# scanner-research/scanner

Measured on AMD Instinct MI355X. Metric: frames/sec (whole node), 1080p histogram + ResNet-50 classify pipelines, higher is better.
Workload: dtype bf16; 1 GPU; model=1080p histogram + ResNet-50 classify, global_batch=512, seq_len=512, parallelism=frame-shard dp1

## Files before the change

### scanner_amd/kernels/gemm_mfma.hip

```cpp
#include <hip/hip_runtime.h>

#include <algorithm>
#include <cstdlib>
#include <map>
#include <mutex>

#include "../csrc/memory.h"
#include "dnn.h"

namespace sca {

namespace {

using bf16 = __bf16;
using bf16x8 = __attribute__((ext_vector_type(8))) __bf16;
using f32x4 = __attribute__((ext_vector_type(4))) float;

__device__ inline float bf16_to_f32(bf16 v) { return (float)v; }

__device__ inline bf16 f32_to_bf16(float v) { return (bf16)v; }

template <int FM, int FN, bool RELU, bool RESIDUAL>
__device__ inline void epilogue_store(f32x4 (&acc)[FM][FN], float* scratch,
                                      bf16* __restrict__ C,
                                      const bf16* __restrict__ residual,
                                      int M, int N, int m0, int n0, int wrow,
                                      int wcol, int lane,
                                      const float* __restrict__ scale,
                                      const float* __restrict__ bias) {
  constexpr int COLS = FN * 16;
  constexpr int STRIDE = COLS + 4;
#pragma unroll
  for (int i = 0; i < FM; ++i) {
    asm volatile("s_waitcnt lgkmcnt(0)");
#pragma unroll
    for (int j = 0; j < FN; ++j) {
      int cw = j * 16 + (lane & 15);
      int col = n0 + wcol * COLS + cw;
      float sc = scale ? scale[col] : 1.f;
      float bi = bias ? bias[col] : 0.f;
#pragma unroll
      for (int r = 0; r < 4; ++r) {
        scratch[((lane >> 4) * 4 + r) * STRIDE + cw] =
            acc[i][j][r] * sc + bi;
      }
    }
    asm volatile("s_waitcnt lgkmcnt(0)");
    constexpr int CHUNK = COLS / 4;
    static_assert(CHUNK >= 8 && CHUNK % 8 == 0, "wave tile too narrow");
    int r2 = lane >> 2;
    int q = lane & 3;
    int row = m0 + wrow * (FM * 16) + i * 16 + r2;
    if (row < M) {
      int colbase = n0 + wcol * COLS + q * CHUNK;
      const float* src = scratch + r2 * STRIDE + q * CHUNK;
      bf16 out[CHUNK];
#pragma unroll
      for (int k = 0; k < CHUNK; ++k) {
        float v = src[k];
        if constexpr (RESIDUAL) {
          v += bf16_to_f32(residual[(size_t)row * N + colbase + k]);
        }
        if constexpr (RELU) v = v > 0.f ? v : 0.f;
        out[k] = f32_to_bf16(v);
      }
#pragma unroll
      for (int c8 = 0; c8 < CHUNK; c8 += 8) {
        *reinterpret_cast<bf16x8*>(C + (size_t)row * N + colbase + c8) =
            *reinterpret_cast<const bf16x8*>(out + c8);
      }
    }
  }
}

template <int BM, int BN, int WM, int WN, bool RELU, bool RESIDUAL,
          bool IMPLICIT>
__global__ void __launch_bounds__(256, 2)
    gemm_bf16_kernel(const bf16* __restrict__ A, const bf16* __restrict__ B,
                     bf16* __restrict__ C, int M, int N, int K,
                     const float* __restrict__ scale,
                     const float* __restrict__ bias,
                     const bf16* __restrict__ residual, ConvDesc d,
                     const bf16* __restrict__ zero) {
  constexpr int BK = 64;
  constexpr int FM = BM / WM / 16;
  constexpr int FN = BN / WN / 16;
  __shared__ bf16 lds[2 * (BM + BN) * BK];

  int tid = threadIdx.x;
  int lane = tid & 63;
  int wave = tid >> 6;
  int wrow = wave / WN;
  int wcol = wave % WN;

  int nwg = gridDim.x;
  int wgid = blockIdx.x;
  if (nwg % 8 == 0) {
    int q = nwg / 8;
    wgid = (wgid % q) * 8 + wgid / q;
  }
  int ntiles_n = (N + BN - 1) / BN;
  int m0 = (wgid / ntiles_n) * BM;
  int n0 = (wgid % ntiles_n) * BN;

  f32x4 acc[FM][FN];
#pragma unroll
  for (int i = 0; i < FM; ++i)
#pragma unroll
    for (int j = 0; j < FN; ++j) acc[i][j] = f32x4{0.f, 0.f, 0.f, 0.f};

  constexpr int A_INSTRS = BM / 8 / 4;
  constexpr int B_INSTRS = BN / 8 / 4;
  const int lrow = lane >> 3;
  const int lk = (lane & 7) * 8;
  i64 imp_rowbase[IMPLICIT ? A_INSTRS : 1];
  int imp_hh0[IMPLICIT ? A_INSTRS : 1];
  int imp_ww0[IMPLICIT ? A_INSTRS : 1];
  int imp_cell = 0, imp_cj = 0, imp_dr = 0, imp_ds = 0;
  if constexpr (IMPLICIT) {
#pragma unroll
    for (int i = 0; i < A_INSTRS; ++i) {
      int row = (wave * A_INSTRS + i) * 8 + lrow;
      int grow = m0 + row;
      if (grow >= M) grow = M - 1;
      int q = grow % d.ow;
      int t = grow / d.ow;
      int p = t % d.oh;
      int nn = t / d.oh;
      imp_rowbase[i] = (i64)nn * d.h * d.w * d.c;
      imp_hh0[i] = p * d.stride - d.pad;
      imp_ww0[i] = q * d.stride - d.pad;
    }
    imp_cell = lk / d.c;
    imp_cj = lk - imp_cell * d.c;
    imp_dr = imp_cell / d.s;
    imp_ds = imp_cell - imp_dr * d.s;
  }
  auto imp_advance = [&](int dk) {
    imp_cj += dk;
    while (imp_cj >= d.c) {
      imp_cj -= d.c;
      ++imp_cell;
      ++imp_ds;
      if (imp_ds == d.s) {
        imp_ds = 0;
        ++imp_dr;
      }
    }
  };
  auto stage = [&](int buf, int k0) {
    bf16* lds_a = lds + buf * (BM + BN) * BK;
    bf16* lds_b = lds_a + BM * BK;
#pragma unroll
    for (int i = 0; i < A_INSTRS; ++i) {
      int row = (wave * A_INSTRS + i) * 8 + lrow;
      int grow = m0 + row;
      if (grow >= M) grow = M - 1;
      const bf16* src;
      if constexpr (IMPLICIT) {
        if (imp_cell >= d.r * d.s) {
          src = zero;
        } else {
          int hh = imp_hh0[i] + imp_dr;
          int ww = imp_ww0[i] + imp_ds;
          src = (hh >= 0 && hh < d.h && ww >= 0 && ww < d.w)
                    ? A + (imp_rowbase[i] + ((i64)hh * d.w + ww) * d.c +
                           imp_cj)
                    : zero;
        }
      } else {
        src = A + (size_t)grow * K + k0 + lk;
      }
      __builtin_amdgcn_global_load_lds(
          (const __attribute__((address_space(1))) uint32_t*)src,
          (__attribute__((address_space(3)))
               uint32_t*)(lds_a + (size_t)(wave * A_INSTRS + i) * 8 * BK),
          16, 0, 0);
    }
#pragma unroll
    for (int i = 0; i < B_INSTRS; ++i) {
      int row = (wave * B_INSTRS + i) * 8 + lrow;
      const bf16* src = B + (size_t)(n0 + row) * K + k0 + lk;
      __builtin_amdgcn_global_load_lds(
          (const __attribute__((address_space(1))) uint32_t*)src,
          (__attribute__((address_space(3)))
               uint32_t*)(lds_b + (size_t)(wave * B_INSTRS + i) * 8 * BK),
          16, 0, 0);
    }
  };

  int ksteps = K / BK;
  stage(0, 0);
  for (int ks = 0; ks < ksteps; ++ks) {
    int buf = ks & 1;
    __builtin_amdgcn_s_waitcnt( 0);
    __syncthreads();
    if (ks + 1 < ksteps) {
      if constexpr (IMPLICIT) imp_advance(BK);
      stage(buf ^ 1, (ks + 1) * BK);
    }

    const bf16* lds_a = lds + buf * (BM + BN) * BK;
    const bf16* lds_b = lds_a + BM * BK;
#pragma unroll
    for (int kk = 0; kk < 2; ++kk) {
      int kbase = kk * 32 + (lane >> 4) * 8;
      bf16x8 afrag[FM], bfrag[FN];
#pragma unroll
      for (int i = 0; i < FM; ++i) {
        int row = wrow * (BM / WM) + i * 16 + (lane & 15);
        afrag[i] = *reinterpret_cast<const bf16x8*>(
            lds_a + (size_t)row * BK + kbase);
      }
#pragma unroll
      for (int j = 0; j < FN; ++j) {
        int col = wcol * (BN / WN) + j * 16 + (lane & 15);
        bfrag[j] = *reinterpret_cast<const bf16x8*>(
            lds_b + (size_t)col * BK + kbase);
      }
#pragma unroll
      for (int i = 0; i < FM; ++i)
#pragma unroll
        for (int j = 0; j < FN; ++j)
          acc[i][j] = __builtin_amdgcn_mfma_f32_16x16x32_bf16(
              afrag[i], bfrag[j], acc[i][j], 0, 0, 0);
    }
  }

  __syncthreads();
  constexpr int EP_STRIDE = BN / WN + 4;
  float* scratch =
      reinterpret_cast<float*>(lds) + (size_t)wave * 16 * EP_STRIDE;
  epilogue_store<FM, FN, RELU, RESIDUAL>(acc, scratch, C, residual, M, N,
                                         m0, n0, wrow, wcol, lane, scale,
                                         bias);
}

template <int BM, int BN, int WM, int WN, bool RELU, bool RESIDUAL>
__global__ void __launch_bounds__(256, 2)
    gemm_bf16_smallk_kernel(const bf16* __restrict__ A,
                            const bf16* __restrict__ B, bf16* __restrict__ C,
                            int M, int N, const float* __restrict__ scale,
                            const float* __restrict__ bias,
                            const bf16* __restrict__ residual,
                            int tiles_per_wg) {
  constexpr int K = 64;
  constexpr int FM = BM / WM / 16;
  constexpr int FN = BN / WN / 16;
  __shared__ bf16 lds_b[BN * K];
  __shared__ bf16 lds_a[2 * BM * K];
  __shared__ float lds_ep[4 * 16 * (BN / WN + 4)];

  int tid = threadIdx.x;
  int lane = tid & 63;
  int wave = tid >> 6;
  int wrow = wave / WN;
  int wcol = wave % WN;

  int ntiles_n = (N + BN - 1) / BN;
  int ntiles_m = (M + BM - 1) / BM;
  int strip = blockIdx.x / ntiles_n;
  int n0 = (blockIdx.x % ntiles_n) * BN;
  int mt0 = strip * tiles_per_wg;
  int mt_end = min(mt0 + tiles_per_wg, ntiles_m);
  if (mt0 >= ntiles_m) return;

  const int lrow = lane >> 3;
  const int lk = (lane & 7) * 8;
  constexpr int B_INSTRS = BN / 8 / 4;
  constexpr int A_INSTRS = BM / 8 / 4;

#pragma unroll
  for (int i = 0; i < B_INSTRS; ++i) {
    int row = (wave * B_INSTRS + i) * 8 + lrow;
    const bf16* src = B + (size_t)(n0 + row) * K + lk;
    __builtin_amdgcn_global_load_lds(
        (const __attribute__((address_space(1))) uint32_t*)src,
        (__attribute__((address_space(3)))
             uint32_t*)(lds_b + (size_t)(wave * B_INSTRS + i) * 8 * K),
        16, 0, 0);
  }

  auto stage_a = [&](int buf, int mt) {
    int m0 = mt * BM;
    bf16* dst = lds_a + buf * BM * K;
#pragma unroll
    for (int i = 0; i < A_INSTRS; ++i) {
      int row = (wave * A_INSTRS + i) * 8 + lrow;
      int grow = m0 + row;
      if (grow >= M) grow = M - 1;
      const bf16* src = A + (size_t)grow * K + lk;
      __builtin_amdgcn_global_load_lds(
          (const __attribute__((address_space(1))) uint32_t*)src,
          (__attribute__((address_space(3)))
               uint32_t*)(dst + (size_t)(wave * A_INSTRS + i) * 8 * K),
          16, 0, 0);
    }
  };

  stage_a(0, mt0);
  for (int mt = mt0; mt < mt_end; ++mt) {
    int buf = (mt - mt0) & 1;
    __builtin_amdgcn_s_waitcnt(0);
    __syncthreads();
    if (mt + 1 < mt_end) stage_a(buf ^ 1, mt + 1);

    f32x4 acc[FM][FN];
#pragma unroll
    for (int i = 0; i < FM; ++i)
#pragma unroll
      for (int j = 0; j < FN; ++j) acc[i][j] = f32x4{0.f, 0.f, 0.f, 0.f};
// ... 11 lines not shown
      }
#pragma unroll
      for (int j = 0; j < FN; ++j) {
        int col = wcol * (BN / WN) + j * 16 + (lane & 15);
        bfrag[j] = *reinterpret_cast<const bf16x8*>(lds_b +
                                                    (size_t)col * K + kbase);
      }
#pragma unroll
      for (int i = 0; i < FM; ++i)
#pragma unroll
        for (int j = 0; j < FN; ++j)
          acc[i][j] = __builtin_amdgcn_mfma_f32_16x16x32_bf16(
              afrag[i], bfrag[j], acc[i][j], 0, 0, 0);
    }

    epilogue_store<FM, FN, RELU, RESIDUAL>(
        acc, lds_ep + (size_t)wave * 16 * (BN / WN + 4), C, residual, M, N,
        mt * BM, n0, wrow, wcol, lane, scale, bias);
  }
}

struct SplitkEp {
  unsigned int* counters = nullptr;
  int splits = 0;
  const float* scale = nullptr;
  const float* bias = nullptr;
  const bf16* residual = nullptr;
  bf16* C = nullptr;
  int relu = 0;
};

template <int BM, int BN, int WM, int WN, bool IMPLICIT, bool ATOMIC>
__global__ void __launch_bounds__(256, 2)
    gemm_bf16_splitk_kernel(const bf16* __restrict__ A,
                            const bf16* __restrict__ B, int M, int N, int K,
                            int ksteps_per_split,
                            float* __restrict__ partials, ConvDesc d,
                            const bf16* __restrict__ zero, SplitkEp ep) {
  constexpr int BK = 64;
  constexpr int FM = BM / WM / 16;
  constexpr int FN = BN / WN / 16;
  __shared__ bf16 lds[2 * (BM + BN) * BK];

  int tid = threadIdx.x;
  int lane = tid & 63;
  int wave = tid >> 6;
  int wrow = wave / WN;
// ... 4 lines not shown
  int tiles = ntiles_m * ntiles_n;
  int split = blockIdx.x / tiles;
  int tile = blockIdx.x % tiles;
  int m0 = (tile / ntiles_n) * BM;
  int n0 = (tile % ntiles_n) * BN;
  int ks_begin = split * ksteps_per_split;
  int ks_end = min(ks_begin + ksteps_per_split, K / BK);
  if (ks_begin >= ks_end) return;

  f32x4 acc[FM][FN];
#pragma unroll
  for (int i = 0; i < FM; ++i)
#pragma unroll
    for (int j = 0; j < FN; ++j) acc[i][j] = f32x4{0.f, 0.f, 0.f, 0.f};

  constexpr int A_INSTRS = BM / 8 / 4;
  constexpr int B_INSTRS = BN / 8 / 4;
  auto stage = [&](int buf, int k0) {
    const int lrow = lane >> 3;
    const int lk = (lane & 7) * 8;
    bf16* lds_a = lds + buf * (BM + BN) * BK;
    bf16* lds_b = lds_a + BM * BK;
#pragma unroll
    for (int i = 0; i < A_INSTRS; ++i) {
      int row = (wave * A_INSTRS + i) * 8 + lrow;
      int grow = m0 + row;
      if (grow >= M) grow = M - 1;
      const bf16* src;
      if constexpr (IMPLICIT) {
        int k = k0 + lk;
        int cell = k / d.c;
        int cj = k - cell * d.c;
        if (cell >= d.r * d.s) {
          src = zero;
        } else {
          int dr = cell / d.s, ds = cell - dr * d.s;
          int q = grow % d.ow;
          int t = grow / d.ow;
          int p = t % d.oh;
          int nn = t / d.oh;
          int hh = p * d.stride - d.pad + dr;
          int ww = q * d.stride - d.pad + ds;
          src = (hh >= 0 && hh < d.h && ww >= 0 && ww < d.w)
                    ? A + ((((i64)nn * d.h + hh) * d.w + ww) * d.c + cj)
                    : zero;
        }
      } else {
        src = A + (size_t)grow * K + k0 + lk;
      }
      __builtin_amdgcn_global_load_lds(
          (const __attribute__((address_space(1))) uint32_t*)src,
          (__attribute__((address_space(3)))
               uint32_t*)(lds_a + (size_t)(wave * A_INSTRS + i) * 8 * BK),
          16, 0, 0);
    }
#pragma unroll
    for (int i = 0; i < B_INSTRS; ++i) {
      int row = (wave * B_INSTRS + i) * 8 + lrow;
      const bf16* src = B + (size_t)(n0 + row) * K + k0 + lk;
      __builtin_amdgcn_global_load_lds(
          (const __attribute__((address_space(1))) uint32_t*)src,
          (__attribute__((address_space(3)))
               uint32_t*)(lds_b + (size_t)(wave * B_INSTRS + i) * 8 * BK),
          16, 0, 0);
    }
  };

  stage(0, ks_begin * BK);
  for (int ks = ks_begin; ks < ks_end; ++ks) {
    int buf = (ks - ks_begin) & 1;
    __builtin_amdgcn_s_waitcnt(0);
    __syncthreads();
    if (ks + 1 < ks_end) stage(buf ^ 1, (ks + 1) * BK);

    const bf16* lds_a = lds + buf * (BM + BN) * BK;
    const bf16* lds_b = lds_a + BM * BK;
#pragma unroll
    for (int kk = 0; kk < 2; ++kk) {
      int kbase = kk * 32 + (lane >> 4) * 8;
      bf16x8 afrag[FM], bfrag[FN];
#pragma unroll
      for (int i = 0; i < FM; ++i) {
        int row = wrow * (BM / WM) + i * 16 + (lane & 15);
        afrag[i] = *reinterpret_cast<const bf16x8*>(
            lds_a + (size_t)row * BK + kbase);
      }
#pragma unroll
      for (int j = 0; j < FN; ++j) {
        int col = wcol * (BN / WN) + j * 16 + (lane & 15);
        bfrag[j] = *reinterpret_cast<const bf16x8*>(
            lds_b + (size_t)col * BK + kbase);
      }
#pragma unroll
      for (int i = 0; i < FM; ++i)
#pragma unroll
        for (int j = 0; j < FN; ++j)
          acc[i][j] = __builtin_amdgcn_mfma_f32_16x16x32_bf16(
              afrag[i], bfrag[j], acc[i][j], 0, 0, 0);
    }
    __syncthreads();
  }

  if constexpr (ATOMIC) {
#pragma unroll
    for (int i = 0; i < FM; ++i) {
#pragma unroll
      for (int j = 0; j < FN; ++j) {
        int col = n0 + wcol * (BN / WN) + j * 16 + (lane & 15);
#pragma unroll
        for (int r = 0; r < 4; ++r) {
          int row = m0 + wrow * (BM / WM) + i * 16 + (lane >> 4) * 4 + r;
          if (row < M)
            atomicAdd(&partials[(size_t)row * N + col], acc[i][j][r]);
        }
      }
// ... 3 lines not shown
#pragma unroll
    for (int i = 0; i < FM; ++i) {
#pragma unroll
      for (int j = 0; j < FN; ++j) {
        int col = n0 + wcol * (BN / WN) + j * 16 + (lane & 15);
#pragma unroll
        for (int r = 0; r < 4; ++r) {
          int row = m0 + wrow * (BM / WM) + i * 16 + (lane >> 4) * 4 + r;
          if (row < M) out[(size_t)row * N + col] = acc[i][j][r];
        }
      }
    }
    if (ep.counters) {
      __threadfence();
      __syncthreads();
      __shared__ unsigned int s_old;
      if (tid == 0) s_old = atomicAdd(ep.counters + tile, 1u);
      __syncthreads();
      if (s_old != (unsigned int)ep.splits - 1) return;
      __threadfence();
      int rows = min(BM, M - m0);
      constexpr int Q = BN / 4;
      for (int idx = tid; idx < rows * Q; idx += 256) {
        int r = idx / Q, q = idx - r * Q;
        size_t base = (size_t)(m0 + r) * N + n0 + q * 4;
        float4 av = make_float4(0.f, 0.f, 0.f, 0.f);
        for (int sp = 0; sp < ep.splits; ++sp) {
          float4 p = *reinterpret_cast<const float4*>(
              partials + (size_t)sp * M * N + base);
          av.x += p.x;
          av.y += p.y;
          av.z += p.z;
          av.w += p.w;
        }
        float v4[4] = {av.x, av.y, av.z, av.w};
        bf16 o4[4];
#pragma unroll
        for (int k = 0; k < 4; ++k) {
          float v = v4[k];
          int col = n0 + q * 4 + k;
          if (ep.scale) v *= ep.scale[col];
          if (ep.bias) v += ep.bias[col];
          if (ep.residual) v += bf16_to_f32(ep.residual[base + k]);
          if (ep.relu) v = v > 0.f ? v : 0.f;
          o4[k] = f32_to_bf16(v);
        }
        *reinterpret_cast<uint64_t*>(ep.C + base) =
            *reinterpret_cast<const uint64_t*>(o4);
      }
      if (tid == 0) ep.counters[tile] = 0;
    }
  }
}

template <bool RELU, bool RESIDUAL>
__global__ void __launch_bounds__(256)
    splitk_finalize_kernel(const float* __restrict__ acc, i64 mn, int N,
                           const float* __restrict__ scale,
                           const float* __restrict__ bias,
                           const bf16* __restrict__ residual,
                           bf16* __restrict__ C) {
  i64 quads = mn / 4;
  i64 gs = (i64)gridDim.x * blockDim.x;
  for (i64 q = (i64)blockIdx.x * blockDim.x + threadIdx.x; q < quads;
       q += gs) {
    i64 i = q * 4;
    float4 a4 = reinterpret_cast<const float4*>(acc)[q];
    float v4[4] = {a4.x, a4.y, a4.z, a4.w};
    bf16 o4[4];
#pragma unroll
    for (int k = 0; k < 4; ++k) {
      float v = v4[k];
      int col = (int)((i + k) % N);
      if (scale) v *= scale[col];
      if (bias) v += bias[col];
      if constexpr (RESIDUAL) v += bf16_to_f32(residual[i + k]);
      if constexpr (RELU) v = v > 0.f ? v : 0.f;
      o4[k] = f32_to_bf16(v);
    }
    *reinterpret_cast<uint64_t*>(C + i) =
        *reinterpret_cast<const uint64_t*>(o4);
  }
}

template <bool RELU, bool RESIDUAL>
__global__ void __launch_bounds__(256)
    splitk_reduce_kernel(const float* __restrict__ partials, int splits,
                         i64 mn, int N, const float* __restrict__ scale,
                         const float* __restrict__ bias,
                         const bf16* __restrict__ residual,
                         bf16* __restrict__ C) {
  i64 quads = mn / 4;
  i64 gs = (i64)gridDim.x * blockDim.x;
  for (i64 q = (i64)blockIdx.x * blockDim.x + threadIdx.x; q < quads;
       q += gs) {
    i64 i = q * 4;
    float4 acc = make_float4(0.f, 0.f, 0.f, 0.f);
    for (int sp = 0; sp < splits; ++sp) {
      float4 p = reinterpret_cast<const float4*>(
          partials + (size_t)sp * mn)[q];
      acc.x += p.x;
      acc.y += p.y;
      acc.z += p.z;
      acc.w += p.w;
    }
    float v4[4] = {acc.x, acc.y, acc.z, acc.w};
    bf16 o4[4];
#pragma unroll
    for (int k = 0; k < 4; ++k) {
      float v = v4[k];
      int col = (int)((i + k) % N);
      if (scale) v *= scale[col];
      if (bias) v += bias[col];
      if constexpr (RESIDUAL) v += bf16_to_f32(residual[i + k]);
      if constexpr (RELU) v = v > 0.f ? v : 0.f;
      o4[k] = f32_to_bf16(v);
    }
    *reinterpret_cast<uint64_t*>(C + i) =
        *reinterpret_cast<const uint64_t*>(o4);
  }
}

const bf16* device_zero_chunk();

constexpr size_t kSplitkCtrBytes = 4096;

bool plan_splitk(int M, int N, int K, size_t scratch_bytes, GemmPlan& p) {
  constexpr int BM = 128, BN = 128;
  static const bool kOff = []() {
    const char* e = std::getenv("SCANNER_SPLITK_OFF");
    return e && e[0] == '1';
  }();
  if (kOff) return false;
  if (!scratch_bytes || N % BN != 0 || K < 1024) return false;
  int ntiles_m = (M + BM - 1) / BM;
  int tiles = ntiles_m * (N / BN);
  if (tiles >= 256) return false;
  static const int kMaxSplits = []() {
// ... 43 lines not shown
        (u8*)g.splitk_scratch + g.splitk_scratch_bytes - kSplitkCtrBytes);
    ep.splits = splits;
    ep.scale = g.scale;
    ep.bias = g.bias;
    ep.residual = (const bf16*)g.residual;
    ep.C = (bf16*)g.C;
    ep.relu = g.relu ? 1 : 0;
  }
  hipError_t e;
  if (kAtomic) {
    e = hipMemsetAsync(g.splitk_scratch, 0, (size_t)mn * 4, s);
    if (e != hipSuccess) {
      throw ScannerError(std::string("splitk memset failed: ") +
                         hipGetErrorString(e));
    }
    if (dd) {
      gemm_bf16_splitk_kernel<BM, BN, 2, 2, true, true>
          <<<grid_main, 256, 0, s>>>(
              (const bf16*)g.A, (const bf16*)g.B, g.M, g.N, g.K,
              ksteps_per_split, (float*)g.splitk_scratch, *dd,
              device_zero_chunk(), SplitkEp{});
    } else {
      gemm_bf16_splitk_kernel<BM, BN, 2, 2, false, true>
          <<<grid_main, 256, 0, s>>>(
              (const bf16*)g.A, (const bf16*)g.B, g.M, g.N, g.K,
              ksteps_per_split, (float*)g.splitk_scratch, ConvDesc{},
              nullptr, SplitkEp{});
    }
  } else if (dd) {
    gemm_bf16_splitk_kernel<BM, BN, 2, 2, true, false>
        <<<grid_main, 256, 0, s>>>(
            (const bf16*)g.A, (const bf16*)g.B, g.M, g.N, g.K,
            ksteps_per_split, (float*)g.splitk_scratch, *dd,
            device_zero_chunk(), ep);
  } else {
    gemm_bf16_splitk_kernel<BM, BN, 2, 2, false, false>
        <<<grid_main, 256, 0, s>>>(
            (const bf16*)g.A, (const bf16*)g.B, g.M, g.N, g.K,
            ksteps_per_split, (float*)g.splitk_scratch, ConvDesc{}, nullptr,
            ep);
  }
  e = hipGetLastError();
  if (e != hipSuccess) {
    throw ScannerError(std::string("splitk launch failed: ") +
                       hipGetErrorString(e));
  }
  if (fused) return;
  int grid = (int)std::min<i64>(4096, (mn + 255) / 256);
  auto disp = [&](auto relu, auto res) {
    if (kAtomic) {
      splitk_finalize_kernel<decltype(relu)::value, decltype(res)::value>
          <<<grid, 256, 0, s>>>((const float*)g.splitk_scratch, mn, g.N,
                                g.scale, g.bias, (const bf16*)g.residual,
                                (bf16*)g.C);
    } else {
      splitk_reduce_kernel<decltype(relu)::value, decltype(res)::value>
          <<<grid, 256, 0, s>>>((const float*)g.splitk_scratch, splits, mn,
                                g.N, g.scale, g.bias,
                                (const bf16*)g.residual, (bf16*)g.C);
    }
  };
  if (g.relu && g.residual)
    disp(std::true_type{}, std::true_type{});
  else if (g.relu)
    disp(std::true_type{}, std::false_type{});
  else if (g.residual)
    disp(std::false_type{}, std::true_type{});
  else
    disp(std::false_type{}, std::false_type{});
  e = hipGetLastError();
  if (e != hipSuccess) {
    throw ScannerError(std::string("splitk reduce launch failed: ") +
                       hipGetErrorString(e));
  }
// ... 33 lines not shown
    disp(std::false_type{}, std::true_type{});
  else
    disp(std::false_type{}, std::false_type{});
  hipError_t e = hipGetLastError();
  if (e != hipSuccess) {
    throw ScannerError(std::string("gemm smallk launch failed: ") +
                       hipGetErrorString(e));
  }
}

template <int BM, int BN, int WM, int WN>
void launch_variant(const GemmArgs& g, hipStream_t s, const GemmPlan& p) {
  const int grid = p.grid;
  auto disp = [&](auto relu, auto res) {
    gemm_bf16_kernel<BM, BN, WM, WN, decltype(relu)::value,
                     decltype(res)::value, false><<<grid, 256, 0, s>>>(
        (const bf16*)g.A, (const bf16*)g.B, (bf16*)g.C, g.M, g.N, g.K,
        g.scale, g.bias, (const bf16*)g.residual, ConvDesc{}, nullptr);
  };
  if (g.relu && g.residual)
    disp(std::true_type{}, std::true_type{});
  else if (g.relu)
    disp(std::true_type{}, std::false_type{});
  else if (g.residual)
    disp(std::false_type{}, std::true_type{});
  else
    disp(std::false_type{}, std::false_type{});
  hipError_t e = hipGetLastError();
  if (e != hipSuccess) {
    throw ScannerError(std::string("gemm launch failed: ") +
                       hipGetErrorString(e));
// ... 10 lines not shown
  if (it != per_dev.end()) return it->second;
  void* p = nullptr;
  hipError_t e = hipMalloc(&p, 256);
  if (e != hipSuccess || hipMemset(p, 0, 256) != hipSuccess) {
    throw ScannerError("failed to allocate implicit-conv zero chunk");
  }
  per_dev[dev] = (bf16*)p;
  return (bf16*)p;
}

template <int BM, int BN, int WM, int WN>
void launch_conv_variant(const GemmArgs& g, const ConvDesc& d,
                         hipStream_t s, const GemmPlan& p) {
  const int grid = p.grid;
  const bf16* zero = device_zero_chunk();
  auto disp = [&](auto relu, auto res) {
    gemm_bf16_kernel<BM, BN, WM, WN, decltype(relu)::value,
                     decltype(res)::value, true><<<grid, 256, 0, s>>>(
        (const bf16*)g.A, (const bf16*)g.B, (bf16*)g.C, g.M, g.N, g.K,
        g.scale, g.bias, (const bf16*)g.residual, d, zero);
  };
  if (g.relu && g.residual)
    disp(std::true_type{}, std::true_type{});
  else if (g.relu)
    disp(std::true_type{}, std::false_type{});
  else if (g.residual)
    disp(std::false_type{}, std::true_type{});
  else
    disp(std::false_type{}, std::false_type{});
  hipError_t e = hipGetLastError();
  if (e != hipSuccess) {
    throw ScannerError(std::string("conv gemm launch failed: ") +
                       hipGetErrorString(e));
  }
}
// ... 75 lines not shown
```

Before: 16280 frames/s.

## Add fast implicit-conv address path, hoist epilogue operands, specialize split-K reduce

```diff
diff --git a/scanner_amd/kernels/gemm_mfma.hip b/scanner_amd/kernels/gemm_mfma.hip
--- a/scanner_amd/kernels/gemm_mfma.hip
+++ b/scanner_amd/kernels/gemm_mfma.hip
@@ -4,6 +4,7 @@
 #include <cstdlib>
 #include <map>
 #include <mutex>
+#include <type_traits>
 
 #include "../csrc/memory.h"
 #include "dnn.h"
@@ -20,14 +21,60 @@
 
 __device__ inline bf16 f32_to_bf16(float v) { return (bf16)v; }
 
+__device__ inline void glds16(const bf16* src, bf16* lds_dst) {
+  __builtin_amdgcn_global_load_lds(
+      (const __attribute__((address_space(1))) uint32_t*)src,
+      (__attribute__((address_space(3))) uint32_t*)lds_dst, 16, 0, 0);
+}
+
+template <int FN>
+__device__ inline void load_scale_bias(float (&sc)[FN], float (&bi)[FN],
+                                       const float* __restrict__ scale,
+                                       const float* __restrict__ bias,
+                                       int col0) {
+  if (scale) {
+#pragma unroll
+    for (int j = 0; j < FN; ++j) sc[j] = scale[col0 + j * 16];
+  } else {
+#pragma unroll
+    for (int j = 0; j < FN; ++j) sc[j] = 1.f;
+  }
+  if (bias) {
+#pragma unroll
+    for (int j = 0; j < FN; ++j) bi[j] = bias[col0 + j * 16];
+  } else {
+#pragma unroll
+    for (int j = 0; j < FN; ++j) bi[j] = 0.f;
+  }
+}
+
+template <int FM, int FN>
+__device__ inline void load_residual(bf16x8 (&res)[FM][FN / 2],
+                                     const bf16* __restrict__ residual,
+                                     int M, int N, int m0, int n0, int wrow,
+                                     int wcol, int lane) {
+  constexpr int COLS = FN * 16;
+  constexpr int CHUNK = COLS / 4;
+  int colbase = n0 + wcol * COLS + (lane & 3) * CHUNK;
+#pragma unroll
+  for (int i = 0; i < FM; ++i) {
+    int row = m0 + wrow * (FM * 16) + i * 16 + (lane >> 2);
+    row = row < M ? row : M - 1;
+    const bf16* src = residual + (size_t)row * N + colbase;
+#pragma unroll
+    for (int c = 0; c < CHUNK / 8; ++c)
+      res[i][c] = *reinterpret_cast<const bf16x8*>(src + c * 8);
+  }
+}
+
 template <int FM, int FN, bool RELU, bool RESIDUAL>
 __device__ inline void epilogue_store(f32x4 (&acc)[FM][FN], float* scratch,
                                       bf16* __restrict__ C,
-                                      const bf16* __restrict__ residual,
-                                      int M, int N, int m0, int n0, int wrow,
+                                      const bf16x8 (&res)[FM][FN / 2], int M,
+                                      int N, int m0, int n0, int wrow,
                                       int wcol, int lane,
-                                      const float* __restrict__ scale,
-                                      const float* __restrict__ bias) {
+                                      const float (&sc)[FN],
+                                      const float (&bi)[FN]) {
   constexpr int COLS = FN * 16;
   constexpr int STRIDE = COLS + 4;
 #pragma unroll
@@ -36,13 +83,10 @@
 #pragma unroll
     for (int j = 0; j < FN; ++j) {
       int cw = j * 16 + (lane & 15);
-      int col = n0 + wcol * COLS + cw;
-      float sc = scale ? scale[col] : 1.f;
-      float bi = bias ? bias[col] : 0.f;
 #pragma unroll
       for (int r = 0; r < 4; ++r) {
         scratch[((lane >> 4) * 4 + r) * STRIDE + cw] =
-            acc[i][j][r] * sc + bi;
+            acc[i][j][r] * sc[j] + bi[j];
       }
     }
     asm volatile("s_waitcnt lgkmcnt(0)");
@@ -58,9 +102,7 @@
 #pragma unroll
       for (int k = 0; k < CHUNK; ++k) {
         float v = src[k];
-        if constexpr (RESIDUAL) {
-          v += bf16_to_f32(residual[(size_t)row * N + colbase + k]);
-        }
+        if constexpr (RESIDUAL) v += bf16_to_f32(res[i][k / 8][k % 8]);
         if constexpr (RELU) v = v > 0.f ? v : 0.f;
         out[k] = f32_to_bf16(v);
       }
@@ -73,8 +115,156 @@
   }
 }
 
+template <int BM, int BN, bool IMPLICIT, bool FAST>
+struct TileStager {
+  static constexpr int BK = 64;
+  static constexpr int A_INSTRS = BM / 8 / 4;
+  static constexpr int B_INSTRS = BN / 8 / 4;
+  static_assert(IMPLICIT || !FAST, "FAST is an implicit-conv mode");
+
+  const bf16* b_src[B_INSTRS];
+  const bf16* a_src[A_INSTRS];
+  uint32_t valid[A_INSTRS];
+  i64 rowbase[A_INSTRS];
+  int hh0[A_INSTRS];
+  int ww0[A_INSTRS];
+  int cell, cj, dr, ds;
+
+  __device__ inline void init(const bf16* __restrict__ A,
+                              const bf16* __restrict__ B, int M, int K,
+                              int m0, int n0, int wave, int lane, int k0,
+                              const ConvDesc& d) {
+    const int lrow = lane >> 3;
+    const int lk = (lane & 7) * 8;
+#pragma unroll
+    for (int i = 0; i < B_INSTRS; ++i) {
+      int row = (wave * B_INSTRS + i) * 8 + lrow;
+      b_src[i] = B + (size_t)(n0 + row) * K + k0 + lk;
+    }
+#pragma unroll
+    for (int i = 0; i < A_INSTRS; ++i) {
+      int row = (wave * A_INSTRS + i) * 8 + lrow;
+      int grow = m0 + row;
+      if (grow >= M) grow = M - 1;
+      if constexpr (!IMPLICIT) {
+        a_src[i] = A + (size_t)grow * K + k0 + lk;
+      } else {
+        int q = grow % d.ow;
+        int t = grow / d.ow;
+        int p = t % d.oh;
+        int nn = t / d.oh;
+        int h0 = p * d.stride - d.pad;
+        int w0 = q * d.stride - d.pad;
+        if constexpr (FAST) {
+          a_src[i] =
+              A + ((((i64)nn * d.h + h0) * d.w + w0) * d.c + lk);
+          uint32_t cmask = 0;
+          for (int x = 0; x < d.s; ++x)
+            cmask |= (uint32_t)((unsigned)(w0 + x) < (unsigned)d.w) << x;
+          uint32_t v = 0;
+          for (int y = 0; y < d.r; ++y)
+            v |= ((unsigned)(h0 + y) < (unsigned)d.h) ? cmask << (y * d.s)
+                                                     : 0u;
+          valid[i] = v;
+        } else {
+          rowbase[i] = (i64)nn * d.h * d.w * d.c;
+          hh0[i] = h0;
+          ww0[i] = w0;
+        }
+      }
+    }
+    if constexpr (IMPLICIT) {
+      int k = FAST ? k0 : k0 + lk;
+      cell = k / d.c;
+      cj = k - cell * d.c;
+      dr = cell / d.s;
+      ds = cell - dr * d.s;
+    }
+  }
+
+  __device__ inline void advance(const ConvDesc& d) {
+#pragma unroll
+    for (int i = 0; i < B_INSTRS; ++i) b_src[i] += BK;
+    if constexpr (!IMPLICIT) {
+#pragma unroll
+      for (int i = 0; i < A_INSTRS; ++i) a_src[i] += BK;
+    } else {
+      cj += BK;
+      while (cj >= d.c) {
+        cj -= d.c;
+        ++cell;
+        ++ds;
+        if (ds == d.s) {
+          ds = 0;
+          ++dr;
+        }
+      }
+    }
+  }
+
+  __device__ inline void issue(bf16* lds_a, int wave,
+                               const bf16* __restrict__ A,
+                               const ConvDesc& d,
+                               const bf16* __restrict__ zero) const {
+    bf16* lds_b = lds_a + BM * BK;
+    i64 step_off = 0;
+    if constexpr (FAST) step_off = ((i64)dr * d.w + ds) * d.c + cj;
+#pragma unroll
+    for (int i = 0; i < A_INSTRS; ++i) {
+      const bf16* src;
+      if constexpr (!IMPLICIT) {
+        src = a_src[i];
+      } else if constexpr (FAST) {
+        src = ((valid[i] >> cell) & 1u) ? a_src[i] + step_off : zero;
+      } else {
+        int hh = hh0[i] + dr;
+        int ww = ww0[i] + ds;
+        bool ok = cell < d.r * d.s && (unsigned)hh < (unsigned)d.h &&
+                  (unsigned)ww < (unsigned)d.w;
+        const bf16* in =
+            A + (rowbase[i] + ((i64)hh * d.w + ww) * d.c + cj);
+        src = ok ? in : zero;
+      }
+      glds16(src, lds_a + (size_t)(wave * A_INSTRS + i) * 8 * BK);
+    }
+#pragma unroll
+    for (int i = 0; i < B_INSTRS; ++i)
+      glds16(b_src[i], lds_b + (size_t)(wave * B_INSTRS + i) * 8 * BK);
+  }
+};
+
+template <int BM, int BN, int WM, int WN, int FM, int FN>
+__device__ inline void mfma_step(f32x4 (&acc)[FM][FN], const bf16* lds_a,
+                                 int wrow, int wcol, int lane) {
+  constexpr int BK = 64;
+  const bf16* lds_b = lds_a + BM * BK;
+#pragma unroll
+  for (int kk = 0; kk < 2; ++kk) {
+    int kbase = kk * 32 + (lane >> 4) * 8;
+    bf16x8 afrag[FM], bfrag[FN];
+#pragma unroll
+    for (int i = 0; i < FM; ++i) {
+      int row = wrow * (BM / WM) + i * 16 + (lane & 15);
+      afrag[i] = *reinterpret_cast<const bf16x8*>(
+          lds_a + (size_t)row * BK + kbase);
+    }
+#pragma unroll
+    for (int j = 0; j < FN; ++j) {
+      int col = wcol * (BN / WN) + j * 16 + (lane & 15);
+      bfrag[j] = *reinterpret_cast<const bf16x8*>(
+          lds_b + (size_t)col * BK + kbase);
+    }
+#pragma unroll
+    for (int i = 0; i < FM; ++i)
+#pragma unroll
+      for (int j = 0; j < FN; ++j)
+        acc[i][j] = __builtin_amdgcn_mfma_f32_16x16x32_bf16(
+            afrag[i], bfrag[j], acc[i][j], 0, 0, 0);
+  }
+}
+
 template <int BM, int BN, int WM, int WN, bool RELU, bool RESIDUAL,
-          bool IMPLICIT>
+          bool IMPLICIT, bool FAST>
 __global__ void __launch_bounds__(256, 2)
     gemm_bf16_kernel(const bf16* __restrict__ A, const bf16* __restrict__ B,
                      bf16* __restrict__ C, int M, int N, int K,
@@ -103,137 +293,44 @@
   int m0 = (wgid / ntiles_n) * BM;
   int n0 = (wgid % ntiles_n) * BN;
 
+  float sc[FN], bi[FN];
+  load_scale_bias<FN>(sc, bi, scale, bias,
+                      n0 + wcol * (FN * 16) + (lane & 15));
+
   f32x4 acc[FM][FN];
 #pragma unroll
   for (int i = 0; i < FM; ++i)
 #pragma unroll
     for (int j = 0; j < FN; ++j) acc[i][j] = f32x4{0.f, 0.f, 0.f, 0.f};
 
-  constexpr int A_INSTRS = BM / 8 / 4;
-  constexpr int B_INSTRS = BN / 8 / 4;
-  const int lrow = lane >> 3;
-  const int lk = (lane & 7) * 8;
-  i64 imp_rowbase[IMPLICIT ? A_INSTRS : 1];
-  int imp_hh0[IMPLICIT ? A_INSTRS : 1];
-  int imp_ww0[IMPLICIT ? A_INSTRS : 1];
-  int imp_cell = 0, imp_cj = 0, imp_dr = 0, imp_ds = 0;
-  if constexpr (IMPLICIT) {
-#pragma unroll
-    for (int i = 0; i < A_INSTRS; ++i) {
-      int row = (wave * A_INSTRS + i) * 8 + lrow;
-      int grow = m0 + row;
-      if (grow >= M) grow = M - 1;
-      int q = grow % d.ow;
-      int t = grow / d.ow;
-      int p = t % d.oh;
-      int nn = t / d.oh;
-      imp_rowbase[i] = (i64)nn * d.h * d.w * d.c;
-      imp_hh0[i] = p * d.stride - d.pad;
-      imp_ww0[i] = q * d.stride - d.pad;
-    }
-    imp_cell = lk / d.c;
-    imp_cj = lk - imp_cell * d.c;
-    imp_dr = imp_cell / d.s;
-    imp_ds = imp_cell - imp_dr * d.s;
-  }
-  auto imp_advance = [&](int dk) {
-    imp_cj += dk;
-    while (imp_cj >= d.c) {
-      imp_cj -= d.c;
-      ++imp_cell;
-      ++imp_ds;
-      if (imp_ds == d.s) {
-        imp_ds = 0;
-        ++imp_dr;
-      }
-    }
-  };
-  auto stage = [&](int buf, int k0) {
-    bf16* lds_a = lds + buf * (BM + BN) * BK;
-    bf16* lds_b = lds_a + BM * BK;
-#pragma unroll
-    for (int i = 0; i < A_INSTRS; ++i) {
-      int row = (wave * A_INSTRS + i) * 8 + lrow;
-      int grow = m0 + row;
-      if (grow >= M) grow = M - 1;
-      const bf16* src;
-      if constexpr (IMPLICIT) {
-        if (imp_cell >= d.r * d.s) {
-          src = zero;
-        } else {
-          int hh = imp_hh0[i] + imp_dr;
-          int ww = imp_ww0[i] + imp_ds;
-          src = (hh >= 0 && hh < d.h && ww >= 0 && ww < d.w)
-                    ? A + (imp_rowbase[i] + ((i64)hh * d.w + ww) * d.c +
-                           imp_cj)
-                    : zero;
-        }
-      } else {
-        src = A + (size_t)grow * K + k0 + lk;
-      }
-      __builtin_amdgcn_global_load_lds(
-          (const __attribute__((address_space(1))) uint32_t*)src,
-          (__attribute__((address_space(3)))
-               uint32_t*)(lds_a + (size_t)(wave * A_INSTRS + i) * 8 * BK),
-          16, 0, 0);
-    }
-#pragma unroll
-    for (int i = 0; i < B_INSTRS; ++i) {
-      int row = (wave * B_INSTRS + i) * 8 + lrow;
-      const bf16* src = B + (size_t)(n0 + row) * K + k0 + lk;
-      __builtin_amdgcn_global_load_lds(
-          (const __attribute__((address_space(1))) uint32_t*)src,
-          (__attribute__((address_space(3)))
-               uint32_t*)(lds_b + (size_t)(wave * B_INSTRS + i) * 8 * BK),
-          16, 0, 0);
-    }
-  };
+  TileStager<BM, BN, IMPLICIT, FAST> st;
+  st.init(A, B, M, K, m0, n0, wave, lane, 0, d);
+  bf16x8 res[FM][FN / 2] = {};
 
   int ksteps = K / BK;
-  stage(0, 0);
-  for (int ks = 0; ks < ksteps; ++ks) {
+  st.issue(lds, wave, A, d, zero);
+  for (int ks = 0; ks + 1 < ksteps; ++ks) {
     int buf = ks & 1;
     __builtin_amdgcn_s_waitcnt( 0);
     __syncthreads();
-    if (ks + 1 < ksteps) {
-      if constexpr (IMPLICIT) imp_advance(BK);
-      stage(buf ^ 1, (ks + 1) * BK);
-    }
-
-    const bf16* lds_a = lds + buf * (BM + BN) * BK;
-    const bf16* lds_b = lds_a + BM * BK;
-#pragma unroll
-    for (int kk = 0; kk < 2; ++kk) {
-      int kbase = kk * 32 + (lane >> 4) * 8;
-      bf16x8 afrag[FM], bfrag[FN];
-#pragma unroll
-      for (int i = 0; i < FM; ++i) {
-        int row = wrow * (BM / WM) + i * 16 + (lane & 15);
-        afrag[i] = *reinterpret_cast<const bf16x8*>(
-            lds_a + (size_t)row * BK + kbase);
-      }
-#pragma unroll
-      for (int j = 0; j < FN; ++j) {
-        int col = wcol * (BN / WN) + j * 16 + (lane & 15);
-        bfrag[j] = *reinterpret_cast<const bf16x8*>(
-            lds_b + (size_t)col * BK + kbase);
-      }
-#pragma unroll
-      for (int i = 0; i < FM; ++i)
-#pragma unroll
-        for (int j = 0; j < FN; ++j)
-          acc[i][j] = __builtin_amdgcn_mfma_f32_16x16x32_bf16(
-              afrag[i], bfrag[j], acc[i][j], 0, 0, 0);
-    }
-  }
+    st.advance(d);
+    st.issue(lds + (buf ^ 1) * (BM + BN) * BK, wave, A, d, zero);
+    mfma_step<BM, BN, WM, WN>(acc, lds + buf * (BM + BN) * BK, wrow, wcol,
+                              lane);
+  }
+  __builtin_amdgcn_s_waitcnt(0);
+  __syncthreads();
+  if constexpr (RESIDUAL)
+    load_residual<FM, FN>(res, residual, M, N, m0, n0, wrow, wcol, lane);
+  mfma_step<BM, BN, WM, WN>(acc, lds + ((ksteps - 1) & 1) * (BM + BN) * BK,
+                            wrow, wcol, lane);
 
   __syncthreads();
   constexpr int EP_STRIDE = BN / WN + 4;
   float* scratch =
       reinterpret_cast<float*>(lds) + (size_t)wave * 16 * EP_STRIDE;
-  epilogue_store<FM, FN, RELU, RESIDUAL>(acc, scratch, C, residual, M, N,
-                                         m0, n0, wrow, wcol, lane, scale,
-                                         bias);
+  epilogue_store<FM, FN, RELU, RESIDUAL>(acc, scratch, C, res, M, N, m0, n0,
+                                         wrow, wcol, lane, sc, bi);
 }
 
 template <int BM, int BN, int WM, int WN, bool RELU, bool RESIDUAL>
@@ -247,9 +344,11 @@
   constexpr int K = 64;
   constexpr int FM = BM / WM / 16;
   constexpr int FN = BN / WN / 16;
-  __shared__ bf16 lds_b[BN * K];
-  __shared__ bf16 lds_a[2 * BM * K];
-  __shared__ float lds_ep[4 * 16 * (BN / WN + 4)];
+  constexpr int EP_FLOATS = 4 * 16 * (BN / WN + 4);
+  __shared__ bf16 lds[BN * K + 2 * BM * K + EP_FLOATS * 2];
+  bf16* lds_b = lds;
+  bf16* lds_a = lds + BN * K;
+  float* lds_ep = reinterpret_cast<float*>(lds + BN * K + 2 * BM * K);
 
   int tid = threadIdx.x;
   int lane = tid & 63;
@@ -265,6 +364,10 @@
   int mt_end = min(mt0 + tiles_per_wg, ntiles_m);
   if (mt0 >= ntiles_m) return;
 
+  float sc[FN], bi[FN];
+  load_scale_bias<FN>(sc, bi, scale, bias,
+                      n0 + wcol * (FN * 16) + (lane & 15));
+
   const int lrow = lane >> 3;
   const int lk = (lane & 7) * 8;
   constexpr int B_INSTRS = BN / 8 / 4;
@@ -273,12 +376,8 @@
 #pragma unroll
   for (int i = 0; i < B_INSTRS; ++i) {
     int row = (wave * B_INSTRS + i) * 8 + lrow;
-    const bf16* src = B + (size_t)(n0 + row) * K + lk;
-    __builtin_amdgcn_global_load_lds(
-        (const __attribute__((address_space(1))) uint32_t*)src,
-        (__attribute__((address_space(3)))
-             uint32_t*)(lds_b + (size_t)(wave * B_INSTRS + i) * 8 * K),
-        16, 0, 0);
+    glds16(B + (size_t)(n0 + row) * K + lk,
+           lds_b + (size_t)(wave * B_INSTRS + i) * 8 * K);
   }
 
   auto stage_a = [&](int buf, int mt) {
@@ -289,12 +388,8 @@
       int row = (wave * A_INSTRS + i) * 8 + lrow;
       int grow = m0 + row;
       if (grow >= M) grow = M - 1;
-      const bf16* src = A + (size_t)grow * K + lk;
-      __builtin_amdgcn_global_load_lds(
-          (const __attribute__((address_space(1))) uint32_t*)src,
-          (__attribute__((address_space(3)))
-               uint32_t*)(dst + (size_t)(wave * A_INSTRS + i) * 8 * K),
-          16, 0, 0);
+      glds16(A + (size_t)grow * K + lk,
+             dst + (size_t)(wave * A_INSTRS + i) * 8 * K);
     }
   };
 
@@ -336,9 +431,13 @@
               afrag[i], bfrag[j], acc[i][j], 0, 0, 0);
     }
 
+    bf16x8 res[FM][FN / 2] = {};
+    if constexpr (RESIDUAL)
+      load_residual<FM, FN>(res, residual, M, N, mt * BM, n0, wrow, wcol,
+                            lane);
     epilogue_store<FM, FN, RELU, RESIDUAL>(
-        acc, lds_ep + (size_t)wave * 16 * (BN / WN + 4), C, residual, M, N,
-        mt * BM, n0, wrow, wcol, lane, scale, bias);
+        acc, lds_ep + (size_t)wave * 16 * (BN / WN + 4), C, res, M, N,
+        mt * BM, n0, wrow, wcol, lane, sc, bi);
   }
 }
 
@@ -352,7 +451,87 @@
   int relu = 0;
 };
 
-template <int BM, int BN, int WM, int WN, bool IMPLICIT, bool ATOMIC>
+template <int S>
+struct SplitPartials {
+  float4 p[S > 0 ? S : 1];
+  const float* base;
+  size_t stride;
+
+  __device__ inline void load(const float* __restrict__ partials,
+                              size_t split_stride, size_t off) {
+    base = partials + off;
+    stride = split_stride;
+#pragma unroll
+    for (int sp = 0; sp < S; ++sp)
+      p[sp] = *reinterpret_cast<const float4*>(base + sp * stride);
+  }
+
+  __device__ inline float4 sum(int splits) const {
+    float4 acc = make_float4(0.f, 0.f, 0.f, 0.f);
+    if constexpr (S > 0) {
+#pragma unroll
+      for (int sp = 0; sp < S; ++sp) {
+        acc.x += p[sp].x;
+        acc.y += p[sp].y;
+        acc.z += p[sp].z;
+        acc.w += p[sp].w;
+      }
+    } else {
+      for (int sp = 0; sp < splits; ++sp) {
+        float4 v = *reinterpret_cast<const float4*>(base + sp * stride);
+        acc.x += v.x;
+        acc.y += v.y;
+        acc.z += v.z;
+        acc.w += v.w;
+      }
+    }
+    return acc;
+  }
+};
+
+struct QuadOperands {
+  float4 sc, bi;
+  uint2 res;
+};
+
+__device__ inline QuadOperands load_quad_operands(
+    const float* __restrict__ scale, const float* __restrict__ bias,
+    const bf16* __restrict__ residual, bool has_res, int col, size_t off) {
+  QuadOperands o;
+  o.sc = make_float4(1.f, 1.f, 1.f, 1.f);
+  o.bi = make_float4(0.f, 0.f, 0.f, 0.f);
+  o.res = make_uint2(0u, 0u);
+  if (scale) o.sc = *reinterpret_cast<const float4*>(scale + col);
+  if (bias) o.bi = *reinterpret_cast<const float4*>(bias + col);
+  if (has_res) o.res = *reinterpret_cast<const uint2*>(residual + off);
+  return o;
+}
+
+__device__ inline void store_quad(float4 a, const QuadOperands& o,
+                                  bool has_scale, bool has_bias,
+                                  bool has_res, bool relu,
+                                  bf16* __restrict__ dst) {
+#pragma clang fp contract(off)
+  float v4[4] = {a.x, a.y, a.z, a.w};
+  float s4[4] = {o.sc.x, o.sc.y, o.sc.z, o.sc.w};
+  float b4[4] = {o.bi.x, o.bi.y, o.bi.z, o.bi.w};
+  bf16 r4[4];
+  *reinterpret_cast<uint2*>(r4) = o.res;
+  bf16 o4[4];
+#pragma unroll
+  for (int k = 0; k < 4; ++k) {
+    float v = v4[k];
+    if (has_scale) v *= s4[k];
+    if (has_bias) v += b4[k];
+    if (has_res) v += bf16_to_f32(r4[k]);
+    if (relu) v = v > 0.f ? v : 0.f;
+    o4[k] = f32_to_bf16(v);
+  }
+  *reinterpret_cast<uint64_t*>(dst) = *reinterpret_cast<const uint64_t*>(o4);
+}
+
+template <int BM, int BN, int WM, int WN, bool IMPLICIT, bool FAST,
+          bool ATOMIC>
 __global__ void __launch_bounds__(256, 2)
     gemm_bf16_splitk_kernel(const bf16* __restrict__ A,
                             const bf16* __restrict__ B, int M, int N, int K,
@@ -387,91 +566,20 @@
 #pragma unroll
     for (int j = 0; j < FN; ++j) acc[i][j] = f32x4{0.f, 0.f, 0.f, 0.f};
 
-  constexpr int A_INSTRS = BM / 8 / 4;
-  constexpr int B_INSTRS = BN / 8 / 4;
-  auto stage = [&](int buf, int k0) {
-    const int lrow = lane >> 3;
-    const int lk = (lane & 7) * 8;
-    bf16* lds_a = lds + buf * (BM + BN) * BK;
-    bf16* lds_b = lds_a + BM * BK;
-#pragma unroll
-    for (int i = 0; i < A_INSTRS; ++i) {
-      int row = (wave * A_INSTRS + i) * 8 + lrow;
-      int grow = m0 + row;
-      if (grow >= M) grow = M - 1;
-      const bf16* src;
-      if constexpr (IMPLICIT) {
-        int k = k0 + lk;
-        int cell = k / d.c;
-        int cj = k - cell * d.c;
-        if (cell >= d.r * d.s) {
-          src = zero;
-        } else {
-          int dr = cell / d.s, ds = cell - dr * d.s;
-          int q = grow % d.ow;
-          int t = grow / d.ow;
-          int p = t % d.oh;
-          int nn = t / d.oh;
-          int hh = p * d.stride - d.pad + dr;
-          int ww = q * d.stride - d.pad + ds;
-          src = (hh >= 0 && hh < d.h && ww >= 0 && ww < d.w)
-                    ? A + ((((i64)nn * d.h + hh) * d.w + ww) * d.c + cj)
-                    : zero;
-        }
-      } else {
-        src = A + (size_t)grow * K + k0 + lk;
-      }
-      __builtin_amdgcn_global_load_lds(
-          (const __attribute__((address_space(1))) uint32_t*)src,
-          (__attribute__((address_space(3)))
-               uint32_t*)(lds_a + (size_t)(wave * A_INSTRS + i) * 8 * BK),
-          16, 0, 0);
-    }
-#pragma unroll
-    for (int i = 0; i < B_INSTRS; ++i) {
-      int row = (wave * B_INSTRS + i) * 8 + lrow;
-      const bf16* src = B + (size_t)(n0 + row) * K + k0 + lk;
-      __builtin_amdgcn_global_load_lds(
-          (const __attribute__((address_space(1))) uint32_t*)src,
-          (__attribute__((address_space(3)))
-               uint32_t*)(lds_b + (size_t)(wave * B_INSTRS + i) * 8 * BK),
-          16, 0, 0);
-    }
-  };
-
-  stage(0, ks_begin * BK);
+  TileStager<BM, BN, IMPLICIT, FAST> st;
+  st.init(A, B, M, K, m0, n0, wave, lane, ks_begin * BK, d);
+
+  st.issue(lds, wave, A, d, zero);
   for (int ks = ks_begin; ks < ks_end; ++ks) {
     int buf = (ks - ks_begin) & 1;
     __builtin_amdgcn_s_waitcnt(0);
     __syncthreads();
-    if (ks + 1 < ks_end) stage(buf ^ 1, (ks + 1) * BK);
-
-    const bf16* lds_a = lds + buf * (BM + BN) * BK;
-    const bf16* lds_b = lds_a + BM * BK;
-#pragma unroll
-    for (int kk = 0; kk < 2; ++kk) {
-      int kbase = kk * 32 + (lane >> 4) * 8;
-      bf16x8 afrag[FM], bfrag[FN];
-#pragma unroll
-      for (int i = 0; i < FM; ++i) {
-        int row = wrow * (BM / WM) + i * 16 + (lane & 15);
-        afrag[i] = *reinterpret_cast<const bf16x8*>(
-            lds_a + (size_t)row * BK + kbase);
-      }
-#pragma unroll
-      for (int j = 0; j < FN; ++j) {
-        int col = wcol * (BN / WN) + j * 16 + (lane & 15);
-        bfrag[j] = *reinterpret_cast<const bf16x8*>(
-            lds_b + (size_t)col * BK + kbase);
-      }
-#pragma unroll
-      for (int i = 0; i < FM; ++i)
-#pragma unroll
-        for (int j = 0; j < FN; ++j)
-          acc[i][j] = __builtin_amdgcn_mfma_f32_16x16x32_bf16(
-              afrag[i], bfrag[j], acc[i][j], 0, 0, 0);
-    }
-    __syncthreads();
+    if (ks + 1 < ks_end) {
+      st.advance(d);
+      st.issue(lds + (buf ^ 1) * (BM + BN) * BK, wave, A, d, zero);
+    }
+    mfma_step<BM, BN, WM, WN>(acc, lds + buf * (BM + BN) * BK, wrow, wcol,
+                              lane);
   }
 
   if constexpr (ATOMIC) {
@@ -505,44 +613,55 @@
     if (ep.counters) {
       __threadfence();
       __syncthreads();
-      __shared__ unsigned int s_old;
+      unsigned int& s_old = *reinterpret_cast<unsigned int*>(lds);
       if (tid == 0) s_old = atomicAdd(ep.counters + tile, 1u);
       __syncthreads();
       if (s_old != (unsigned int)ep.splits - 1) return;
       __threadfence();
       int rows = min(BM, M - m0);
       constexpr int Q = BN / 4;
+      const size_t mn = (size_t)M * N;
       for (int idx = tid; idx < rows * Q; idx += 256) {
         int r = idx / Q, q = idx - r * Q;
         size_t base = (size_t)(m0 + r) * N + n0 + q * 4;
-        float4 av = make_float4(0.f, 0.f, 0.f, 0.f);
-        for (int sp = 0; sp < ep.splits; ++sp) {
-          float4 p = *reinterpret_cast<const float4*>(
-              partials + (size_t)sp * M * N + base);
-          av.x += p.x;
-          av.y += p.y;
-          av.z += p.z;
-          av.w += p.w;
+        auto finish = [&](auto nsplit) {
+          SplitPartials<decltype(nsplit)::value> sp;
+          sp.load(partials, mn, base);
+          QuadOperands o =
+              load_quad_operands(ep.scale, ep.bias, ep.residual,
+                                 ep.residual != nullptr, n0 + q * 4, base);
+          store_quad(sp.sum(ep.splits), o, ep.scale != nullptr,
+                     ep.bias != nullptr, ep.residual != nullptr,
+                     ep.relu != 0, ep.C + base);
+        };
+        switch (ep.splits) {
+          case 2: finish(std::integral_constant<int, 2>{}); break;
+          case 3: finish(std::integral_constant<int, 3>{}); break;
+          case 4: finish(std::integral_constant<int, 4>{}); break;
+          case 5: finish(std::integral_constant<int, 5>{}); break;
+          case 6: finish(std::integral_constant<int, 6>{}); break;
+          default: finish(std::integral_constant<int, 0>{});
         }
-        float v4[4] = {av.x, av.y, av.z, av.w};
-        bf16 o4[4];
-#pragma unroll
-        for (int k = 0; k < 4; ++k) {
-          float v = v4[k];
-          int col = n0 + q * 4 + k;
-          if (ep.scale) v *= ep.scale[col];
-          if (ep.bias) v += ep.bias[col];
-          if (ep.residual) v += bf16_to_f32(ep.residual[base + k]);
-          if (ep.relu) v = v > 0.f ? v : 0.f;
-          o4[k] = f32_to_bf16(v);
-        }
-        *reinterpret_cast<uint64_t*>(ep.C + base) =
-            *reinterpret_cast<const uint64_t*>(o4);
       }
       if (tid == 0) ep.counters[tile] = 0;
     }
   }
 }
+
+struct QuadColumn {
+  unsigned nq, cq, cstep;
+  __device__ inline QuadColumn(int N) {
+    nq = (unsigned)N / 4;
+    unsigned gs = gridDim.x * blockDim.x;
+    cq = (blockIdx.x * blockDim.x + threadIdx.x) % nq;
+    cstep = gs % nq;
+  }
+  __device__ inline int col() const { return (int)(cq * 4); }
+  __device__ inline void next() {
+    cq += cstep;
+    if (cq >= nq) cq -= nq;
+  }
+};
 
 template <bool RELU, bool RESIDUAL>
 __global__ void __launch_bounds__(256)
@@ -553,28 +672,19 @@
                            bf16* __restrict__ C) {
   i64 quads = mn / 4;
   i64 gs = (i64)gridDim.x * blockDim.x;
+  QuadColumn qc(N);
   for (i64 q = (i64)blockIdx.x * blockDim.x + threadIdx.x; q < quads;
-       q += gs) {
+       q += gs, qc.next()) {
     i64 i = q * 4;
     float4 a4 = reinterpret_cast<const float4*>(acc)[q];
-    float v4[4] = {a4.x, a4.y, a4.z, a4.w};
-    bf16 o4[4];
-#pragma unroll
-    for (int k = 0; k < 4; ++k) {
-      float v = v4[k];
-      int col = (int)((i + k) % N);
-      if (scale) v *= scale[col];
-      if (bias) v += bias[col];
-      if constexpr (RESIDUAL) v += bf16_to_f32(residual[i + k]);
-      if constexpr (RELU) v = v > 0.f ? v : 0.f;
-      o4[k] = f32_to_bf16(v);
-    }
-    *reinterpret_cast<uint64_t*>(C + i) =
-        *reinterpret_cast<const uint64_t*>(o4);
-  }
-}
-
-template <bool RELU, bool RESIDUAL>
+    QuadOperands o = load_quad_operands(scale, bias, residual, RESIDUAL,
+                                        qc.col(), (size_t)i);
+    store_quad(a4, o, scale != nullptr, bias != nullptr, RESIDUAL, RELU,
+               C + i);
+  }
+}
+
+template <bool RELU, bool RESIDUAL, int S>
 __global__ void __launch_bounds__(256)
     splitk_reduce_kernel(const float* __restrict__ partials, int splits,
                          i64 mn, int N, const float* __restrict__ scale,
@@ -583,36 +693,24 @@
                          bf16* __restrict__ C) {
   i64 quads = mn / 4;
   i64 gs = (i64)gridDim.x * blockDim.x;
+  QuadColumn qc(N);
   for (i64 q = (i64)blockIdx.x * blockDim.x + threadIdx.x; q < quads;
-       q += gs) {
+       q += gs, qc.next()) {
     i64 i = q * 4;
-    float4 acc = make_float4(0.f, 0.f, 0.f, 0.f);
-    for (int sp = 0; sp < splits; ++sp) {
-      float4 p = reinterpret_cast<const float4*>(
-          partials + (size_t)sp * mn)[q];
-      acc.x += p.x;
-      acc.y += p.y;
-      acc.z += p.z;
-      acc.w += p.w;
-    }
-    float v4[4] = {acc.x, acc.y, acc.z, acc.w};
-    bf16 o4[4];
-#pragma unroll
-    for (int k = 0; k < 4; ++k) {
-      float v = v4[k];
-      int col = (int)((i + k) % N);
-      if (scale) v *= scale[col];
-      if (bias) v += bias[col];
-      if constexpr (RESIDUAL) v += bf16_to_f32(residual[i + k]);
-      if constexpr (RELU) v = v > 0.f ? v : 0.f;
-      o4[k] = f32_to_bf16(v);
-    }
-    *reinterpret_cast<uint64_t*>(C + i) =
-        *reinterpret_cast<const uint64_t*>(o4);
+    SplitPartials<S> sp;
+    sp.load(partials, (size_t)mn, (size_t)i);
+    QuadOperands o = load_quad_operands(scale, bias, residual, RESIDUAL,
+                                        qc.col(), (size_t)i);
+    store_quad(sp.sum(splits), o, scale != nullptr, bias != nullptr,
+               RESIDUAL, RELU, C + i);
   }
 }
 
 const bf16* device_zero_chunk();
+
+bool conv_fast_path(const ConvDesc& d, int K) {
+  return d.c % 64 == 0 && d.r * d.s <= 32 && K == d.r * d.s * d.c;
+}
 
 constexpr size_t kSplitkCtrBytes = 4096;
 
@@ -686,32 +784,30 @@
       throw ScannerError(std::string("splitk memset failed: ") +
                          hipGetErrorString(e));
     }
-    if (dd) {
-      gemm_bf16_splitk_kernel<BM, BN, 2, 2, true, true>
-          <<<grid_main, 256, 0, s>>>(
-              (const bf16*)g.A, (const bf16*)g.B, g.M, g.N, g.K,
-              ksteps_per_split, (float*)g.splitk_scratch, *dd,
-              device_zero_chunk(), SplitkEp{});
-    } else {
-      gemm_bf16_splitk_kernel<BM, BN, 2, 2, false, true>
-          <<<grid_main, 256, 0, s>>>(
-              (const bf16*)g.A, (const bf16*)g.B, g.M, g.N, g.K,
-              ksteps_per_split, (float*)g.splitk_scratch, ConvDesc{},
-              nullptr, SplitkEp{});
-    }
-  } else if (dd) {
-    gemm_bf16_splitk_kernel<BM, BN, 2, 2, true, false>
+  }
+  auto main_kernel = [&](auto implicit, auto fast, auto atomic) {
+    constexpr bool kImplicit = decltype(implicit)::value;
+    gemm_bf16_splitk_kernel<BM, BN, 2, 2, kImplicit, decltype(fast)::value,
+                            decltype(atomic)::value>
         <<<grid_main, 256, 0, s>>>(
             (const bf16*)g.A, (const bf16*)g.B, g.M, g.N, g.K,
-            ksteps_per_split, (float*)g.splitk_scratch, *dd,
-            device_zero_chunk(), ep);
-  } else {
-    gemm_bf16_splitk_kernel<BM, BN, 2, 2, false, false>
-        <<<grid_main, 256, 0, s>>>(
-            (const bf16*)g.A, (const bf16*)g.B, g.M, g.N, g.K,
-            ksteps_per_split, (float*)g.splitk_scratch, ConvDesc{}, nullptr,
-            ep);
-  }
+            ksteps_per_split, (float*)g.splitk_scratch,
+            kImplicit ? *dd : ConvDesc{},
+            kImplicit ? device_zero_chunk() : nullptr,
+            decltype(atomic)::value ? SplitkEp{} : ep);
+  };
+  auto by_atomic = [&](auto implicit, auto fast) {
+    if (kAtomic)
+      main_kernel(implicit, fast, std::true_type{});
+    else
+      main_kernel(implicit, fast, std::false_type{});
+  };
+  if (!dd)
+    by_atomic(std::false_type{}, std::false_type{});
+  else if (conv_fast_path(*dd, g.K))
+    by_atomic(std::true_type{}, std::true_type{});
+  else
+    by_atomic(std::true_type{}, std::false_type{});
   e = hipGetLastError();
   if (e != hipSuccess) {
     throw ScannerError(std::string("splitk launch failed: ") +
@@ -726,10 +822,21 @@
                                 g.scale, g.bias, (const bf16*)g.residual,
                                 (bf16*)g.C);
     } else {
-      splitk_reduce_kernel<decltype(relu)::value, decltype(res)::value>
-          <<<grid, 256, 0, s>>>((const float*)g.splitk_scratch, splits, mn,
-                                g.N, g.scale, g.bias,
-                                (const bf16*)g.residual, (bf16*)g.C);
+      auto reduce = [&](auto nsplit) {
+        splitk_reduce_kernel<decltype(relu)::value, decltype(res)::value,
+                             decltype(nsplit)::value>
+            <<<grid, 256, 0, s>>>((const float*)g.splitk_scratch, splits, mn,
+                                  g.N, g.scale, g.bias,
+                                  (const bf16*)g.residual, (bf16*)g.C);
+      };
+      switch (splits) {
+        case 2: reduce(std::integral_constant<int, 2>{}); break;
+        case 3: reduce(std::integral_constant<int, 3>{}); break;
+        case 4: reduce(std::integral_constant<int, 4>{}); break;
+        case 5: reduce(std::integral_constant<int, 5>{}); break;
+        case 6: reduce(std::integral_constant<int, 6>{}); break;
+        default: reduce(std::integral_constant<int, 0>{});
+      }
     }
   };
   if (g.relu && g.residual)
@@ -793,7 +900,8 @@
   const int grid = p.grid;
   auto disp = [&](auto relu, auto res) {
     gemm_bf16_kernel<BM, BN, WM, WN, decltype(relu)::value,
-                     decltype(res)::value, false><<<grid, 256, 0, s>>>(
+                     decltype(res)::value, false, false>
+        <<<grid, 256, 0, s>>>(
         (const bf16*)g.A, (const bf16*)g.B, (bf16*)g.C, g.M, g.N, g.K,
         g.scale, g.bias, (const bf16*)g.residual, ConvDesc{}, nullptr);
   };
@@ -834,11 +942,19 @@
                          hipStream_t s, const GemmPlan& p) {
   const int grid = p.grid;
   const bf16* zero = device_zero_chunk();
+  const bool fast = conv_fast_path(d, g.K);
+  auto launch = [&](auto relu, auto res, auto fast_t) {
+    gemm_bf16_kernel<BM, BN, WM, WN, decltype(relu)::value,
+                     decltype(res)::value, true, decltype(fast_t)::value>
+        <<<grid, 256, 0, s>>>(
+            (const bf16*)g.A, (const bf16*)g.B, (bf16*)g.C, g.M, g.N, g.K,
+            g.scale, g.bias, (const bf16*)g.residual, d, zero);
+  };
   auto disp = [&](auto relu, auto res) {
-    gemm_bf16_kernel<BM, BN, WM, WN, decltype(relu)::value,
-                     decltype(res)::value, true><<<grid, 256, 0, s>>>(
-        (const bf16*)g.A, (const bf16*)g.B, (bf16*)g.C, g.M, g.N, g.K,
-        g.scale, g.bias, (const bf16*)g.residual, d, zero);
+    if (fast)
+      launch(relu, res, std::true_type{});
+    else
+      launch(relu, res, std::false_type{});
   };
   if (g.relu && g.residual)
     disp(std::true_type{}, std::true_type{});
```

After: 18060 frames/s (median of 6 runs). +10.9%, better.
